# yuyuyu-bot/various_image_processings

Hardware: AMD Instinct MI355X
Metric: Mpixels/sec bilateral r=7 on 4K RGB; % HBM roofline; 1/2/4/8-GPU scaling (higher is better)
Workload: dtype f32; 1 GPU; bilateral r=7 3840x2160 RGB8; ksize=15, frame=3840x2160, rows_per_rank=2160, data=uniform, parallelism=row-tiled x1

## Files before the change

### include/vip.h

```cpp
#ifndef VIP_H
#define VIP_H

#include <stddef.h>
#include <stdint.h>

#ifdef __cplusplus
extern "C" {
#endif

#define VIP_ABI_VERSION 1

#define VIP_NUMERICS_CUDA 0
#define VIP_NUMERICS_CPP 1

#define VIP_ERR_INVALID_ARGUMENT 10001
#define VIP_ERR_UNSUPPORTED_KSIZE 10002
#define VIP_ERR_ALIASING 10003

typedef struct vip_bilateral_s* vip_bilateral_t;
typedef struct vip_adaptive_s* vip_adaptive_t;
typedef struct vip_texture_s* vip_texture_t;
typedef struct vip_upsample_s* vip_upsample_t;

int vip_abi_version(void);
// ... 55 lines not shown
                                 int row_hi, int free_cus, void* stream);
int vip_bilateral_run_c1(vip_bilateral_t h, const uint8_t* d_src, size_t src_pitch, uint8_t* d_dst, size_t dst_pitch,
                         void* stream);
int vip_joint_bilateral_run_c1(vip_bilateral_t h, const uint8_t* d_src, size_t src_pitch, const uint8_t* d_guide,
                               size_t guide_pitch, int guide_channels, uint8_t* d_dst, size_t dst_pitch,
                               void* stream);
int vip_bilateral_run_rows_c1(vip_bilateral_t h, const uint8_t* d_src, size_t src_pitch, const uint8_t* d_guide,
                              size_t guide_pitch, int guide_channels, uint8_t* d_dst, size_t dst_pitch, int out_rows,
                              int src_row0, int row_lo, int row_hi, void* stream);
int vip_joint_bilateral_run_f32(vip_bilateral_t h, const float* d_src, size_t src_pitch, const uint8_t* d_guide,
                                size_t guide_pitch, int guide_channels, float* d_dst, size_t dst_pitch,
                                void* stream);
int vip_joint_bilateral_run_rows_f32(vip_bilateral_t h, const float* d_src, size_t src_pitch,
                                     const uint8_t* d_guide, size_t guide_pitch, int guide_channels, float* d_dst,
                                     size_t dst_pitch, int out_rows, int src_row0, int row_lo, int row_hi,
                                     void* stream);
int vip_joint_bilateral_run_conf_f32(vip_bilateral_t h, const float* d_src, size_t src_pitch, const float* d_conf,
                                     size_t conf_pitch, const uint8_t* d_guide, size_t guide_pitch,
                                     int guide_channels, float hole_value, float* d_dst, size_t dst_pitch,
                                     float* d_weight , size_t weight_pitch, void* stream);
int vip_joint_bilateral_run_f32c(vip_bilateral_t h, const float* d_src, size_t src_pitch, int channels,
                                 const uint8_t* d_guide, size_t guide_pitch, int guide_channels, float* d_dst,
                                 size_t dst_pitch, void* stream);
int vip_upsample_create(vip_upsample_t* out, int width, int height, int scale, int ksize, float sigma_space,
                        float sigma_color, int numerics);
int vip_upsample_destroy(vip_upsample_t h);
int vip_upsample_low_size(int width, int height, int scale, int* low_width, int* low_height);
int vip_upsample_run_f32(vip_upsample_t h, const float* d_src_lo, size_t src_pitch, const uint8_t* d_guide_lo,
                         size_t guide_lo_pitch, const uint8_t* d_guide, size_t guide_pitch, int guide_channels,
                         float* d_dst, size_t dst_pitch, void* stream);
int vip_bilateral_set_waves(int waves);
int vip_bilateral_set_wide(int mode);
int vip_bilateral_set_frames_in_flight(int n);

int vip_adaptive_create(vip_adaptive_t* out, int width, int height, int ksize, float sigma_space, float sigma_color,
                        int numerics);
int vip_adaptive_destroy(vip_adaptive_t h);
int vip_adaptive_run(vip_adaptive_t h, const uint8_t* d_src, size_t src_pitch, uint8_t* d_dst, size_t dst_pitch,
                     void* stream);
int vip_adaptive_run_rows(vip_adaptive_t h, const uint8_t* d_src, size_t src_pitch, uint8_t* d_dst, size_t dst_pitch,
                          int out_rows, int src_row0, int row_lo, int row_hi, void* stream);
int vip_adaptive_run_rows_batch(vip_adaptive_t h, int n, const uint8_t* const* d_srcs, size_t src_pitch,
                                uint8_t* const* d_dsts, size_t dst_pitch, int out_rows, int src_row0, int row_lo,
                                int row_hi, int free_cus, void* stream);
int vip_adaptive_run_c1(vip_adaptive_t h, const uint8_t* d_src, size_t src_pitch, uint8_t* d_dst, size_t dst_pitch,
                        void* stream);
int vip_adaptive_run_rows_c1(vip_adaptive_t h, const uint8_t* d_src, size_t src_pitch, uint8_t* d_dst,
                             size_t dst_pitch, int out_rows, int src_row0, int row_lo, int row_hi, void* stream);

int vip_gradient_u8(const uint8_t* d_src, float* d_dst, int width, int height, int src_ch, int numerics,
                    void* stream);
int vip_gradient_f32(const float* d_src, float* d_dst, int width, int height, int src_ch, int numerics,
                     void* stream);

int vip_texture_create(vip_texture_t* out, int width, int height, int ksize, int nitr, int numerics);
int vip_texture_destroy(vip_texture_t h);
size_t vip_texture_scratch_bytes(int width, int height);
int vip_texture_run(vip_texture_t h, const uint8_t* d_src, uint8_t* d_dst, void* stream);
int vip_texture_run_timed(vip_texture_t h, const uint8_t* d_src, uint8_t* d_dst, void* stream, void* const* events);

#define VIP_TEXTURE_TWO_LAUNCH 0
#define VIP_TEXTURE_FUSED 1
int vip_texture_set_mode(vip_texture_t h, int mode);

int vip_texture_run_c1(vip_texture_t h, const uint8_t* d_src, size_t src_pitch, uint8_t* d_dst, size_t dst_pitch,
                       void* stream);
// ... 14 lines not shown
```

### various_image_processings_amd/_lib.py

```python
from __future__ import annotations

import ctypes
import os
import threading

_HERE = os.path.dirname(os.path.abspath(__file__))
LIB_PATH = os.path.join(_HERE, "libvip_hip.so")

VIP_NUMERICS_CUDA = 0
VIP_NUMERICS_CPP = 1
VIP_ERR_INVALID_ARGUMENT = 10001
VIP_ERR_UNSUPPORTED_KSIZE = 10002
VIP_ERR_ALIASING = 10003
VIP_FILTER_BILATERAL, VIP_FILTER_JOINT, VIP_FILTER_ADAPTIVE, VIP_FILTER_TEXTURE = 0, 1, 2, 3
VIP_FILTER_UPSAMPLE = 4
VIP_FILTER_JOINT_CONF = 5
VIP_FILTER_JOINT_F32C = 6
VIP_PATH_AUTO, VIP_PATH_RUNTIME = 0, 1

_c_void_p = ctypes.c_void_p
_c_int = ctypes.c_int
_c_float = ctypes.c_float
_c_size_t = ctypes.c_size_t

# ... 57 lines not shown
        _c_int, [_c_void_p, _c_void_p, _c_size_t, _c_int, _c_void_p, _c_size_t, _c_int, _c_void_p, _c_size_t,
                 _c_void_p]),
    "vip_joint_f32c_max_ksize": (_c_int, [_c_int]),
    "vip_upsample_create": (
        _c_int, [ctypes.POINTER(_c_void_p), _c_int, _c_int, _c_int, _c_int, _c_float, _c_float, _c_int]),
    "vip_upsample_destroy": (_c_int, [_c_void_p]),
    "vip_upsample_low_size": (_c_int, [_c_int, _c_int, _c_int, ctypes.POINTER(_c_int), ctypes.POINTER(_c_int)]),
    "vip_upsample_run_f32": (
        _c_int, [_c_void_p, _c_void_p, _c_size_t, _c_void_p, _c_size_t, _c_void_p, _c_size_t, _c_int,
                 _c_void_p, _c_size_t, _c_void_p]),
    "vip_adaptive_create": (_c_int, [ctypes.POINTER(_c_void_p), _c_int, _c_int, _c_int, _c_float, _c_float, _c_int]),
    "vip_adaptive_destroy": (_c_int, [_c_void_p]),
    "vip_adaptive_run": (_c_int, [_c_void_p, _c_void_p, _c_size_t, _c_void_p, _c_size_t, _c_void_p]),
    "vip_adaptive_run_rows": (
        _c_int, [_c_void_p, _c_void_p, _c_size_t, _c_void_p, _c_size_t, _c_int, _c_int, _c_int, _c_int, _c_void_p]),
    "vip_adaptive_run_rows_batch": (
        _c_int, [_c_void_p, _c_int, ctypes.POINTER(_c_void_p), _c_size_t, ctypes.POINTER(_c_void_p), _c_size_t,
                 _c_int, _c_int, _c_int, _c_int, _c_int, _c_void_p]),
    "vip_adaptive_run_c1": (_c_int, [_c_void_p, _c_void_p, _c_size_t, _c_void_p, _c_size_t, _c_void_p]),
    "vip_adaptive_run_rows_c1": (
        _c_int, [_c_void_p, _c_void_p, _c_size_t, _c_void_p, _c_size_t, _c_int, _c_int, _c_int, _c_int, _c_void_p]),
    "vip_gradient_u8": (_c_int, [_c_void_p, _c_void_p, _c_int, _c_int, _c_int, _c_int, _c_void_p]),
    "vip_gradient_f32": (_c_int, [_c_void_p, _c_void_p, _c_int, _c_int, _c_int, _c_int, _c_void_p]),
    "vip_texture_create": (_c_int, [ctypes.POINTER(_c_void_p), _c_int, _c_int, _c_int, _c_int, _c_int]),
    "vip_texture_destroy": (_c_int, [_c_void_p]),
    "vip_texture_run": (_c_int, [_c_void_p, _c_void_p, _c_void_p, _c_void_p]),
    "vip_texture_run_timed": (_c_int, [_c_void_p, _c_void_p, _c_void_p, _c_void_p, ctypes.POINTER(_c_void_p)]),
    "vip_texture_run_c1": (_c_int, [_c_void_p, _c_void_p, _c_size_t, _c_void_p, _c_size_t, _c_void_p]),
    "vip_texture_halo_rows": (_c_int, [_c_int]),
    "vip_texture_set_mode": (_c_int, [_c_void_p, _c_int]),
    "vip_bilateral_set_waves": (_c_int, [_c_int]),
    "vip_bilateral_set_wide": (_c_int, [_c_int]),
    "vip_bilateral_set_frames_in_flight": (_c_int, [_c_int]),
    "vip_texture_iterate_rows": (_c_int, [_c_void_p, _c_void_p, _c_void_p, _c_size_t, _c_int, _c_int, _c_int, _c_int,
                                          _c_void_p]),
    "vip_texture_blur_rtv": (_c_int, [_c_void_p, _c_void_p, _c_void_p, _c_void_p, _c_void_p, _c_void_p]),
    "vip_texture_guide": (_c_int, [_c_void_p, _c_void_p, _c_void_p, _c_void_p, _c_void_p]),
}

_lock = threading.Lock()
_lib = None


class VipError(RuntimeError):

    def __init__(self, func: str, code: int):
        self.code = code
        msg = lib().vip_error_string(code).decode()
        super().__init__(f"{func} failed with status {code}: {msg}")


def lib() -> ctypes.CDLL:
    global _lib
    with _lock:
        if _lib is None:
            if not os.path.exists(LIB_PATH):
                raise ImportError(
                    f"{LIB_PATH} is not built; run __graft_entry__.build() "
                    "(make -C various_image_processings_amd/csrc)")
            handle = ctypes.CDLL(LIB_PATH)
            for name, (res, args) in SIGNATURES.items():
                fn = getattr(handle, name)
                fn.restype = res
                fn.argtypes = args
            _lib = handle
    return _lib
# ... 10 lines not shown
```

### various_image_processings_amd/csrc/vip_bilateral.hip

```cpp
#include "vip_launch.hpp"
#include "vip_stencil.hpp"

namespace vip {

#ifdef VIP_STAMPS
__device__ unsigned long long vip_stamps[256 * 16 * 8 * 3];
__device__ __forceinline__ void vip_stamp(int blk, int wave, int t, int k) {
    if ((threadIdx.x & 63) == 0 && t < 8 && blk < 256)
        vip_stamps[((blk * 16 + wave) * 8 + t) * 3 + k] = __builtin_amdgcn_s_memtime();
}
#define VIP_STAMP(t, k) vip_stamp(blockIdx.x, wave, t, k)
__device__ unsigned long long vip_rt[256 * 4];
__device__ __forceinline__ void vip_rt_stamp(int k) {
    if (threadIdx.x == 0 && blockIdx.x < 256) {
        vip_rt[blockIdx.x * 4 + 2 * k] = __builtin_amdgcn_s_memtime();
        vip_rt[blockIdx.x * 4 + 2 * k + 1] = __builtin_amdgcn_s_memrealtime();
    }
}
#define VIP_RT_STAMP(k) vip_rt_stamp(k)
#else
#define VIP_STAMP(t, k)
#define VIP_RT_STAMP(k)
#endif

constexpr int kBilUnrollMaxR = 15;
constexpr bool kBilRcp = true;
template <int R>
struct FoldRank {
    int t[(R + 1) * (R + 1)];
    constexpr FoldRank() : t() {
        for (int y = 0; y <= R; ++y)
            for (int x = 0; x <= R; ++x) t[y * (R + 1) + x] = disc_r2_rank(R, x * x + y * y);
    }
};
constexpr int kPairShareDist = 3;
template <int R, int WAVES, bool JOINT, bool FMA, int COPIES, int P, int NE, bool FOLD, int TPR, bool SAT, bool MULTI>
__device__ __forceinline__ void bilateral_body(const StencilArgs& a) {
    using G = Geom<R, P, TPR>;
    constexpr int NT = WAVES * 64;
    constexpr int TH = WAVES * G::RPW;
    constexpr bool ROW_UNROLL = R <= kBilUnrollMaxR;
    constexpr int ROWS = TH + 2 * R;
    constexpr int PLANE = ROWS * G::S;
    extern __shared__ __attribute__((aligned(16))) uint32_t lds[];
    uint32_t* const lut = lds;
    constexpr int NTAB = FOLD ? disc_r2_count(R) : 1;
    static_assert(SAT == FOLD, "the saturating address serves the folded tables only");
    static_assert(!FOLD || (NE == 32 && COPIES == sat_fold_copies<R>()), "folded tables: saturating address");
    using SL = SatLut<R, 4 * (JOINT ? 2 : 1) * PLANE, disc_r2_count(R), kSatFoldDz, COPIES>;
    uint32_t* const gplane = SAT ? lds + SL::PL / 4 : lds + NTAB * NE * COPIES;
    uint32_t* const splane = JOINT ? gplane + PLANE : gplane;

    const int tid = threadIdx.x;
    const int lane = tid & 63;
    const int wave = __builtin_amdgcn_readfirstlane(tid >> 6);
    const int tx = lane % TPR;
    const int ty = wave * G::RPW + lane / TPR;
    const uint32_t lane4 = (uint32_t)(lane & (COPIES - 1)) << 2;
    const uint32_t sbias = (uint32_t)SL::B0 + lane4;
    const char* const lut_bytes = reinterpret_cast<const char*>(lut);
    const float w0 = __uint_as_float(__builtin_amdgcn_readfirstlane(
        __float_as_uint(FOLD ? a.fold[disc_r2_rank(R, 0) * kFoldEntries] : a.color[0] * a.ws[0])));

    VIP_RT_STAMP(0);
    int tile = blockIdx.x;
    const int items = launch_items<MULTI>(a);
    TilePrefetch<R, ROWS, NT, P, TPR> pg, ps;
    std::conditional_t<SAT, SatStage<NT, SL>, LutStage<NT, NTAB * NE, COPIES>> ls;
    ls.load(FOLD ? a.fold : a.color);
    {
        const FrameTile ft = frame_tile<MULTI>(a, item_tile<MULTI>(a, tile));
        const int tx0 = (ft.t % a.tiles_x) * G::TW, ty0 = (ft.t / a.tiles_x) * TH;
        pg.issue(JOINT ? a.guide : frame_src<MULTI>(a.guide, ft.f), a.guide_pitch, a, tx0, ty0);
        if constexpr (JOINT) ps.issue(a.src, a.src_pitch, a, tx0, ty0);
    }
    ls.store(SAT ? lds + SL::T / 4 : lut);
    pg.commit(gplane);
    if constexpr (JOINT) ps.commit(splane);
    __syncthreads();

    for ([[maybe_unused]] int it = 0;; ++it) {
        VIP_STAMP(it, 0);
        const FrameTile ft = frame_tile<MULTI>(a, item_tile<MULTI>(a, tile));
        const int tx0 = (ft.t % a.tiles_x) * G::TW, ty0 = (ft.t / a.tiles_x) * TH;
        const int next = tile + (int)gridDim.x;
        if (next < items) {
            const FrameTile fn = frame_tile<MULTI>(a, item_tile<MULTI>(a, next));
            const int nx0 = (fn.t % a.tiles_x) * G::TW, ny0 = (fn.t / a.tiles_x) * TH;
            pg.issue(JOINT ? a.guide : frame_src<MULTI>(a.guide, fn.f), a.guide_pitch, a, nx0, ny0);
            if constexpr (JOINT) ps.issue(a.src, a.src_pitch, a, nx0, ny0);
        }
        if (ty0 + wave * G::RPW < a.out_rows && item_wave<MULTI, WAVES>(a, tile, wave)) {
            uint32_t ctr[P];
            {
                const uint4* c = reinterpret_cast<const uint4*>(gplane + (ty + R) * G::S + tx * P + G::L);
#pragma unroll
                for (int q = 0; q < P / 4; ++q) {
                    const uint4 v = c[q];
                    ctr[4 * q + 0] = v.x; ctr[4 * q + 1] = v.y; ctr[4 * q + 2] = v.z; ctr[4 * q + 3] = v.w;
                }
            }
            f2 a01[P], a2k[P];
#pragma unroll
            for (int i = 0; i < P; ++i) a01[i] = a2k[i] = f2{0.f, 0.f};

            for_each_row<R, ROW_UNROLL>([&](const int ky, auto hwc) {
                    constexpr int HW = decltype(hwc)::value;
                    const int aky = ky < 0 ? -ky : ky;
                    set_progress_priority((ky + R) * 4 / (2 * R + 1));
                    const int row_off = (ty + R + ky) * G::S + tx * P;
                    const float* const ws = a.ws + aky * kWsStride;
                    constexpr int C0 = (G::L - HW) / 4, C1 = (G::L + P - 1 + HW) / 4;
                    constexpr int NC = C1 - C0 + 1;
                    float wsv[HW + 1];
#pragma unroll
                    for (int k = 0; k <= HW; ++k) wsv[k] = ws[k];
                    auto widx = [&](uint32_t g, f2, f2, int i, int kx) {
                        uint32_t d = __builtin_amdgcn_sad_u8(g, ctr[i], 0u);
                        if constexpr (FOLD) {
                            constexpr FoldRank<R> rank;
                            return sat_addr(d, SL::S, sbias) + (uint32_t)(SL::T - SL::B0) +
                                   4u * COPIES * rank.t[aky * (R + 1) + (kx < 0 ? -kx : kx)];
                        }
                        return (d << (COPIES == 32 ? 7 : 6)) | lane4;
                    };
// ... 24 lines not shown
        tile = next;
    }
}

template <int R, int WAVES, bool JOINT, bool FMA, int COPIES, int P, int NE = 768, bool FOLD = false, int TPR = 16,
          bool SAT = false>
__global__ __launch_bounds__(WAVES * 64) void bilateral_kernel(const StencilArgs a) {
    bilateral_body<R, WAVES, JOINT, FMA, COPIES, P, NE, FOLD, TPR, SAT, false>(a);
}
template <int R, int WAVES, bool JOINT, bool FMA, int COPIES, int P, int NE = 768, bool FOLD = false, int TPR = 16,
          bool SAT = false>
__global__ __launch_bounds__(WAVES * 64) void bilateral_frames_kernel(const StencilArgs a) {
    bilateral_body<R, WAVES, JOINT, FMA, COPIES, P, NE, FOLD, TPR, SAT, true>(a);
}

constexpr bool kJbfLut16 = true;
constexpr int kJbfP8MaxR = 7;
constexpr int kBilP = 8;
template <int R, int PLANES>
constexpr int outputs_per_thread() { return PLANES == 2 ? (R <= kJbfP8MaxR ? 8 : 4) : kBilP; }
template <int R, int PLANES>
constexpr int lut_copies() {
    constexpr int P = outputs_per_thread<R, PLANES>();
    if (!kJbfLut16 || PLANES == 1) return 32;
    return pick_waves<R, PLANES, 16, 768 * 16, P>() > pick_waves<R, PLANES, 16, 768 * 32, P>() ? 16 : 32;
}

constexpr int kBilSmallMaxR = 8;
constexpr float kWideWork = 0.55f;
struct Tiling {
    int waves;
    bool wide;
};
inline Tiling small_frame_tiling(int width, int out_rows, int inflight = 1, int nframes = 1) {
    const int forced = bilateral_forced_waves();
    const int fwide = bilateral_forced_wide();
    const int share = device_cus() / (inflight > 1 ? inflight : 1);
    const int cus = share > 0 ? share : 1;
    const int cand[3] = {16, 8, 4};
    const float cost[3] = {1.0f, 1.25f, 1.8f};
    Tiling best{16, false};
    float best_t = 0.f;
    bool first = true;
    for (int wide = 0; wide < 2; ++wide) {
        if ((fwide == 1 && wide) || (fwide == 2 && !wide) || (fwide == 0 && forced && wide)) continue;
        const int tw = wide ? 256 : 128, rpw = wide ? 1 : 4;
        const long long tiles_x = (width + tw - 1) / tw;
        for (int i = 0; i < 3; ++i) {
            if (forced && cand[i] != forced) continue;
            const int th = cand[i] * rpw;
            const long long tiles = tiles_x * ((out_rows + th - 1) / th) * (nframes > 1 ? nframes : 1);
            const float t = (float)((tiles + cus - 1) / cus) * cand[i] * cost[i] * (wide ? kWideWork : 1.f);
            if (first || t < best_t) best = Tiling{cand[i], wide != 0}, best_t = t, first = false;
        }
    }
    return best;
}

template <int R, bool JOINT, bool FMA, bool FOLD, int WAVES, bool WIDE = false>
static int launch_bilateral_w(const StencilArgs& a, hipStream_t stream);

template <int R, int WAVES, int PLANES, int P>
constexpr int sat_lds_bytes() {
    return SatLut<R, 4 * PLANES * (WAVES * Geom<R, P>::RPW + 2 * R) * Geom<R, P>::S, disc_r2_count(R), kSatFoldDz,
                  sat_fold_copies<R>()>::BYTES;
}
template <int R, int PLANES, int P>
constexpr int pick_waves_sat() {
    if (sat_lds_bytes<R, 16, PLANES, P>() <= kLdsBudget) return 16;
    if (sat_lds_bytes<R, 12, PLANES, P>() <= kLdsBudget) return 12;
    if (sat_lds_bytes<R, 8, PLANES, P>() <= kLdsBudget) return 8;
    return sat_lds_bytes<R, 4, PLANES, P>() <= kLdsBudget ? 4 : 0;
}

template <int R, bool JOINT, bool FMA, bool FOLD>
static int launch_bilateral_lut(const StencilArgs& a, hipStream_t stream) {
    constexpr int PLANES = JOINT ? 2 : 1;
    constexpr int P = outputs_per_thread<R, PLANES>();
    constexpr int WAVES = FOLD ? pick_waves_sat<R, PLANES, P>()
                               : pick_waves<R, PLANES, 16, 768 * lut_copies<R, PLANES>(), P>();
    static_assert(WAVES > 0, "tile does not fit LDS");
    if constexpr (!JOINT && WAVES == 16 && R <= kBilSmallMaxR) {
        const Tiling t = small_frame_tiling(a.width, a.out_rows, a.inflight, a.nframes);
        if (t.wide) {
            if (t.waves == 16) return launch_bilateral_w<R, JOINT, FMA, FOLD, 16, true>(a, stream);
            if (t.waves == 8) return launch_bilateral_w<R, JOINT, FMA, FOLD, 8, true>(a, stream);
            return launch_bilateral_w<R, JOINT, FMA, FOLD, 4, true>(a, stream);
        }
        if (t.waves == 8) return launch_bilateral_w<R, JOINT, FMA, FOLD, 8>(a, stream);
        if (t.waves == 4) return launch_bilateral_w<R, JOINT, FMA, FOLD, 4>(a, stream);
    }
    return launch_bilateral_w<R, JOINT, FMA, FOLD, WAVES>(a, stream);
}

template <int R, bool JOINT, bool FMA, bool FOLD, int WAVES, bool WIDE>
static int launch_bilateral_w(const StencilArgs& a, hipStream_t stream) {
    static_assert(!FOLD || JOINT, "folded tables: the joint filter");
    static_assert(!WIDE || !JOINT, "wide tiles: the plain filter");
    constexpr int PLANES = JOINT ? 2 : 1;
    constexpr int P = WIDE ? 4 : outputs_per_thread<R, PLANES>();
    constexpr int TPR = WIDE ? 64 : 16;
    using G = Geom<R, P, TPR>;
    constexpr int NE = FOLD ? kFoldEntries : 768;
    constexpr int COPIES = FOLD ? sat_fold_copies<R>() : lut_copies<R, PLANES>();
    constexpr int TH = WAVES * G::RPW;
    constexpr int LDS = FOLD ? sat_lds_bytes<R, WAVES, PLANES, P>() : lds_bytes<R, WAVES, PLANES, NE * COPIES, P, TPR>();
    static_assert(LDS <= kLdsBudget, "tile does not fit LDS");
    constexpr bool SAT = FOLD;
    constexpr auto kern = bilateral_kernel<R, WAVES, JOINT, FMA, COPIES, P, NE, FOLD, TPR, SAT>;
    if constexpr (!JOINT && R <= kBatchMaxRadius) {
        constexpr auto frames_kern = bilateral_frames_kernel<R, WAVES, JOINT, FMA, COPIES, P, NE, FOLD, TPR, SAT>;
        return launch_persistent<kern, frames_kern, LDS, WAVES, G::TW, TH, SAT>(a, a.inflight <= 1, stream);
    } else {
        if (!JOINT && a.nframes > 1) return VIP_ERR_INVALID_ARGUMENT;
        return launch_persistent<kern, nullptr, LDS, WAVES, G::TW, TH, SAT>(a, false, stream);
    }
}

template <int R, bool JOINT, bool FMA>
static int launch_bilateral_r(const StencilArgs& a, hipStream_t stream) {
    if constexpr (JOINT && R <= kSatMaxR)
        if (a.fold && a.lut_nonzero <= SatLut<R, 0, disc_r2_count(R), kSatFoldDz, sat_fold_copies<R>()>::DZ)
            return launch_bilateral_lut<R, JOINT, FMA, true>(a, stream);
    return launch_bilateral_lut<R, JOINT, FMA, false>(a, stream);
}

template <bool JOINT, bool FMA>
static int launch_bilateral_dispatch(int radius, const StencilArgs& a, hipStream_t stream) {
    switch (radius) {
#define VIP_CASE(RR) \
    case RR: return launch_bilateral_r<RR, JOINT, FMA>(a, stream);
#ifdef VIP_ONLY_R7
        VIP_CASE(4) VIP_CASE(7) VIP_CASE(15)
#else
        VIP_CASE(1) VIP_CASE(2) VIP_CASE(3) VIP_CASE(4) VIP_CASE(5) VIP_CASE(6) VIP_CASE(7) VIP_CASE(8)
        VIP_CASE(9) VIP_CASE(10) VIP_CASE(11) VIP_CASE(12) VIP_CASE(13) VIP_CASE(14) VIP_CASE(15)
#endif
#undef VIP_CASE
        default: return VIP_ERR_UNSUPPORTED_KSIZE;
    }
}

#if defined(VIP_BIL_JOINT) && defined(VIP_BIL_FMA)
int launch_bilateral_joint_fma(int radius, const StencilArgs& a, hipStream_t s) {
    return launch_bilateral_dispatch<true, true>(radius, a, s);
}
#elif defined(VIP_BIL_JOINT)
int launch_bilateral_joint_mul(int radius, const StencilArgs& a, hipStream_t s) {
    return launch_bilateral_dispatch<true, false>(radius, a, s);
}
#elif defined(VIP_BIL_FMA)
int launch_bilateral_plain_fma(int radius, const StencilArgs& a, hipStream_t s) {
    return launch_bilateral_dispatch<false, true>(radius, a, s);
}
#ifdef VIP_STAMPS
}
extern "C" int vip_debug_read_stamps(void* host, size_t bytes) {
    return (int)hipMemcpyFromSymbol(host, HIP_SYMBOL(vip::vip_stamps), bytes, 0, hipMemcpyDeviceToHost);
}
extern "C" int vip_debug_read_rt(void* host, size_t bytes) {
    return (int)hipMemcpyFromSymbol(host, HIP_SYMBOL(vip::vip_rt), bytes, 0, hipMemcpyDeviceToHost);
}
namespace vip {
#endif
#else
int launch_bilateral_plain_mul(int radius, const StencilArgs& a, hipStream_t s) {
    return launch_bilateral_dispatch<false, false>(radius, a, s);
}
#endif

}
```

### various_image_processings_amd/csrc/vip_capi.hip

```cpp
#include <atomic>
#include <cmath>
#include <cstdlib>
#include <cstdio>
#include <cstring>
#include <cxxabi.h>
#include <dlfcn.h>
#include <new>
#include <string>
#include <vector>

#include "vip_launch.hpp"

namespace vip {
static int launch_stencil(int filter, int radius, bool fma, const StencilArgs& a, hipStream_t s) {
    if (filter == VIP_FILTER_JOINT)
        return fma ? launch_bilateral_joint_fma(radius, a, s) : launch_bilateral_joint_mul(radius, a, s);
    if (filter == VIP_FILTER_ADAPTIVE) return fma ? launch_adaptive_fma(radius, a, s) : launch_adaptive_mul(radius, a, s);
    return fma ? launch_bilateral_plain_fma(radius, a, s) : launch_bilateral_plain_mul(radius, a, s);
}

static float space_weight(int r2, float sigma_space, int numerics) {
    const float two_s2 = 2 * sigma_space * sigma_space;
    const float cf = -1.f / two_s2;
    const double cd = -1. / (double)two_s2;
// ... 393 lines not shown
        case VIP_FILTER_UPSAMPLE: return kMaxKsizeUpsample;
        case VIP_FILTER_JOINT_CONF: return kMaxKsizeJointConf;
        case VIP_FILTER_JOINT_F32C: return kMaxKsizeJointF32c[2];
        default: return VIP_ERR_INVALID_ARGUMENT;
    }
}

int vip_joint_f32c_max_ksize(int channels) {
    return channels >= 1 && channels <= 4 ? kMaxKsizeJointF32c[channels] : VIP_ERR_INVALID_ARGUMENT;
}

int vip_set_stencil_path(int path) {
    if (path != VIP_PATH_AUTO && path != VIP_PATH_RUNTIME) return VIP_ERR_INVALID_ARGUMENT;
    g_stencil_path.store(path, std::memory_order_relaxed);
    return 0;
}

int vip_bilateral_set_waves(int waves) {
    if (!valid_waves(waves)) return VIP_ERR_INVALID_ARGUMENT;
    g_bil_waves.store(waves, std::memory_order_relaxed);
    return 0;
}

int vip_bilateral_set_wide(int mode) {
    if (mode < 0 || mode > 2) return VIP_ERR_INVALID_ARGUMENT;
    g_bil_wide.store(mode, std::memory_order_relaxed);
    return 0;
}

int vip_bilateral_set_frames_in_flight(int n) {
    if (n < 0 || n > 4) return VIP_ERR_INVALID_ARGUMENT;
    g_bil_inflight.store(n, std::memory_order_relaxed);
    return 0;
}

const char* vip_error_string(int code) {
    switch (code) {
        case 0: return "success";
        case VIP_ERR_INVALID_ARGUMENT: return "invalid argument";
        case VIP_ERR_UNSUPPORTED_KSIZE:
            return "unsupported ksize (odd, 1..65 bilateral, 1..47 joint bilateral, 1..63 adaptive, 1..9 upsampling, 1..31 confidence-weighted "
                   "joint, 1..31 / 1..15 joint on 2 / 3-4 f32 channels; texture 1..24)";
        case VIP_ERR_ALIASING: return "source and destination alias";
        default: return hipGetErrorString((hipError_t)code);
    }
}

int vip_malloc(void** d_ptr, size_t bytes) {
    if (!d_ptr) return VIP_ERR_INVALID_ARGUMENT;
    return (int)hipMalloc(d_ptr, bytes);
}
int vip_free(void* d_ptr) { return (int)hipFree(d_ptr); }
int vip_upload(void* d_dst, const void* h_src, size_t bytes) {
    return (int)hipMemcpy(d_dst, h_src, bytes, hipMemcpyHostToDevice);
}
int vip_download(void* h_dst, const void* d_src, size_t bytes) {
    return (int)hipMemcpy(h_dst, d_src, bytes, hipMemcpyDeviceToHost);
}
int vip_device_synchronize(void) { return (int)hipDeviceSynchronize(); }
int vip_device_count(int* count) {
    if (!count) return VIP_ERR_INVALID_ARGUMENT;
    return (int)hipGetDeviceCount(count);
}
int vip_set_device(int device) { return (int)hipSetDevice(device); }
int vip_get_device(int* device) {
    if (!device) return VIP_ERR_INVALID_ARGUMENT;
// ... 592 lines not shown
```

### various_image_processings_amd/csrc/vip_launch.hpp

```cpp
#pragma once

#include <atomic>
#include <type_traits>
#include <utility>

#include <hip/hip_ext.h>

#include "vip_common.hpp"

namespace vip {

constexpr int kMaxRadius = 15;
constexpr int kWsStride = kMaxRadius + 1;
constexpr int kP = 8;
constexpr int kTW = 16 * kP;
constexpr int kLdsBudget = 160 * 1024;
constexpr int kSatMaxR = 6;
constexpr int kFoldEntries = 32;

constexpr int kMaxBatchFrames = 6;
constexpr int kBatchMaxRadius = 8;

struct StencilArgs {
    const uint8_t* src;
// ... 11 lines not shown
    const float* color;
    int lut_nonzero;
    const float* fold;
    int inflight;
    int nframes;
    int tiles_frame;
    int free_cus;
    int tail_full, tail_shift;
    const uint8_t* fsrc[kMaxBatchFrames];
    uint8_t* fdst[kMaxBatchFrames];
    float ws[kWsStride * kWsStride];
};

constexpr int kRtMaxRadius = 32;

struct RtArgs {
    const uint8_t* src;
    const uint8_t* guide;
    uint8_t* dst;
    long long src_pitch, guide_pitch, dst_pitch;
    int width, out_rows, src_row0, row_lo, row_hi;
    int aligned, dst_aligned;
    const float* color;
    const float* wsrow;
    const int* hw;
    int R, wst, ra;
    int L, S, tiles_x;
};

int launch_bilateral_joint_fma(int radius, const StencilArgs& a, hipStream_t s);
int launch_bilateral_joint_mul(int radius, const StencilArgs& a, hipStream_t s);
int launch_bilateral_plain_fma(int radius, const StencilArgs& a, hipStream_t s);
int launch_bilateral_plain_mul(int radius, const StencilArgs& a, hipStream_t s);
int launch_adaptive_fma(int radius, const StencilArgs& a, hipStream_t s);
int launch_adaptive_mul(int radius, const StencilArgs& a, hipStream_t s);
int launch_stencil_rt(const RtArgs& a, bool joint, bool adaptive, bool fma, hipStream_t stream);
int launch_gray(int radius, int guide_channels, bool fma, const StencilArgs& a, hipStream_t s);
int launch_gray_rt(const RtArgs& a, int guide_channels, bool fma, hipStream_t s);
int launch_gray_adaptive(int radius, bool fma, const StencilArgs& a, hipStream_t s);
int launch_gray_adaptive_rt(const RtArgs& a, bool fma, hipStream_t s);
constexpr int kF32GuideWords = 1;
constexpr int kF32SrcVec = 2;
int launch_joint_f32(int radius, int guide_channels, bool fma, const StencilArgs& a, hipStream_t s);
int launch_joint_f32_rt(const RtArgs& a, int guide_channels, bool fma, hipStream_t s);
constexpr int kUpMaxRadius = 4;
constexpr int kUpGuideWords = 4;
struct UpsampleArgs {
    const uint8_t* src;
    const uint8_t* guide_lo;
    const uint8_t* guide;
    uint8_t* dst;
    long long src_pitch, guide_lo_pitch, guide_pitch, dst_pitch;
    int width, out_rows;
    int low_width, low_height;
    int tiles_x, tiles_total;
    int aligned, dst_aligned;
    const float* color;
    const float* wsp;
};
int launch_upsample_f32(int radius, int scale, int guide_channels, bool fma, const UpsampleArgs& a, hipStream_t s);
struct ConfArgs : StencilArgs {
    const uint8_t* conf;
    uint8_t* weight;
    long long conf_pitch, weight_pitch;
    float hole_value;
    int conf_vec;
// ... 136 lines not shown
```

### various_image_processings_amd/csrc/vip_stencil.hpp

```cpp
#pragma once

#include <type_traits>
#include <utility>

#include "vip_exact.hpp"
#include "vip_launch.hpp"

namespace vip {

constexpr int kSatFoldDz = kFoldEntries - 1;
static_assert(kSatFoldDz < kFoldEntries, "folded tables hold d < kFoldEntries");

template <int R, int PB, int NTAB_ = disc_r2_count(R), int DZMAX = kSatFoldDz, int COPIES_ = 32>
struct SatLut {
    static constexpr int NTAB = NTAB_;
    static constexpr int COPIES = COPIES_;
    static constexpr int S = NTAB * 4 * COPIES;
    static constexpr int LAST = 4 * (COPIES - 1);
    static constexpr int DZ = (65535 - LAST) / S < DZMAX ? (65535 - LAST) / S : DZMAX;
    static constexpr int B0 = 65535 - DZ * S - LAST;
    static constexpr int T = round_up(B0, 16);
    static constexpr int PL = PB <= B0 ? 0 : round_up(T + (DZ + 1) * S, 16);
    static constexpr int BYTES = PB <= B0 ? T + (DZ + 1) * S : PL + PB;
    static_assert(COPIES == 16 || COPIES == 32, "copies");
    static_assert(DZ >= 0 && T - B0 + (NTAB - 1) * 4 * COPIES <= 65535, "ds_read immediate range");
};
template <int R>
constexpr int sat_fold_copies() { return R <= 6 ? 32 : 16; }
static_assert(SatLut<6, 0>::DZ >= 25 && SatLut<8, 0, disc_r2_count(8), kSatFoldDz, 16>::DZ >= 25 &&
                  SatLut<7, 0, disc_r2_count(7), kSatFoldDz, 32>::DZ < 25,
              "folded tables reach the texture JBF's zero point (d = 25) with sat_fold_copies");

constexpr int lut_words(bool adaptive) { return adaptive ? 1536 * 16 : 768 * 32; }

__device__ __forceinline__ int xcd_tile(int slot, int total) {
    const int grid = (int)gridDim.x, b = (int)blockIdx.x;
    const int base = slot - b;
    if ((grid & 7) != 0 || base + grid > total) return slot;
    return base + (b & 7) * (grid >> 3) + (b >> 3);
}

template <int R, int P = kP, int TPR = 16>
struct Geom {
    static_assert((P == 8 && TPR == 16) || (P == 4 && (TPR == 16 || TPR == 64)), "P, TPR");
    static constexpr int TW = TPR * P;
    static constexpr int RPW = 64 / TPR;
    static constexpr int L = round_up(R, 4);
    static constexpr int S = P == 8 ? round_up(TW + 2 * L, 8) + 4
                                    : (TPR == 64 ? round_up(TW + 2 * L, 4) : round_up(TW + 2 * L, 64));
    static constexpr int GROUPS = (TW + 2 * L) / 4;
};

template <int R, int WAVES, int PLANES, int LUTW = lut_words(false), int P = kP, int TPR = 16>
constexpr int lds_bytes() {
    return 4 * LUTW + 4 * PLANES * (WAVES * Geom<R, P, TPR>::RPW + 2 * R) * Geom<R, P, TPR>::S;
}

template <int R, int PLANES, int MAXW = 16, int LUTW = lut_words(false), int P = kP, int TPR = 16>
constexpr int pick_waves() {
    if (MAXW >= 16 && lds_bytes<R, 16, PLANES, LUTW, P, TPR>() <= kLdsBudget) return 16;
    if (MAXW >= 12 && lds_bytes<R, 12, PLANES, LUTW, P, TPR>() <= kLdsBudget) return 12;
    if (MAXW >= 8 && lds_bytes<R, 8, PLANES, LUTW, P, TPR>() <= kLdsBudget) return 8;
    return MAXW >= 4 && lds_bytes<R, 4, PLANES, LUTW, P, TPR>() <= kLdsBudget ? 4 : 0;
}

template <int R, int KY>
struct HwDispatch {
    template <class F>
    __device__ __forceinline__ static void run(int hw, F&& f) {
        constexpr int H = circle_hw(R, KY);
        if constexpr (KY == 0 || circle_hw(R, KY - 1) != H) {
            if (hw == H) {
                f(std::integral_constant<int, H>{});
                return;
            }
        }
        if constexpr (KY < R) HwDispatch<R, KY + 1>::run(hw, static_cast<F&&>(f));
    }
};

template <int R, bool UNROLL, class F>
__device__ __forceinline__ void for_each_row(F&& f) {
    if constexpr (UNROLL) {
        [&]<int... I>(std::integer_sequence<int, I...>) {
// ... 5 lines not shown
            const int aky = ky < 0 ? -ky : ky;
            HwDispatch<R, 0>::run(circle_hw(R, aky), [&](auto hwc) { f(ky, hwc); });
        }
    }
}

__device__ __forceinline__ uint4 unpack_rgb4(uint32_t a, uint32_t b, uint32_t c) {
    uint4 r;
    r.x = a & 0xffffffu;
    r.y = __builtin_amdgcn_alignbyte(b, a, 3) & 0xffffffu;
    r.z = __builtin_amdgcn_alignbyte(c, b, 2) & 0xffffffu;
    r.w = c >> 8;
    return r;
}

__device__ __forceinline__ uint32_t load_rgb(const uint8_t* row, int x) {
    const uint8_t* p = row + 3 * x;
    return (uint32_t)p[0] | ((uint32_t)p[1] << 8) | ((uint32_t)p[2] << 16);
}

template <int N, int K>
__device__ __forceinline__ void win_sum(const uint32_t (&x)[N + K - 1], uint32_t (&o)[N]) {
    uint32_t s = x[0];
#pragma unroll
    for (int k = 1; k < K; ++k) s += x[k];
    o[0] = s;
#pragma unroll
    for (int j = 1; j < N; ++j) {
        s = s + x[j + K - 1] - x[j - 1];
        o[j] = s;
    }
}

template <int R, int ROWS, int NT, int P = kP, int TPR = 16>
struct TilePrefetch {
    using G = Geom<R, P, TPR>;
    static constexpr int NG = ROWS * G::GROUPS;
    static constexpr int K = (NG + NT - 1) / NT;
    uint32_t raw[K][3];

    __device__ __forceinline__ void issue(const uint8_t* img, long long pitch, const StencilArgs& a, int tx0,
                                          int ty0) {
#pragma unroll
        for (int k = 0; k < K; ++k) {
            const int g = (int)threadIdx.x + k * NT;
            if (NG % NT != 0 && k == K - 1 && g >= NG) continue;
            const int r = g / G::GROUPS;
            const int gc = g - r * G::GROUPS;
            const int sy = clampi(ty0 + a.src_row0 - R + r, a.row_lo, a.row_hi - 1);
            const uint8_t* row = img + (long long)sy * pitch;
            const int x = tx0 - G::L + 4 * gc;
            if (a.aligned && x >= 0 && x + 3 < a.width) {
                const uint32_t* w = reinterpret_cast<const uint32_t*>(row + 3 * x);
                raw[k][0] = w[0];
                raw[k][1] = w[1];
                raw[k][2] = w[2];
            } else {
                const uint32_t q0 = load_rgb(row, clampi(x + 0, 0, a.width - 1));
                const uint32_t q1 = load_rgb(row, clampi(x + 1, 0, a.width - 1));
                const uint32_t q2 = load_rgb(row, clampi(x + 2, 0, a.width - 1));
                const uint32_t q3 = load_rgb(row, clampi(x + 3, 0, a.width - 1));
                raw[k][0] = q0 | (q1 << 24);
                raw[k][1] = (q1 >> 8) | (q2 << 16);
                raw[k][2] = (q2 >> 16) | (q3 << 8);
            }
        }
    }

    __device__ __forceinline__ void commit(uint32_t* plane) const {
// ... 150 lines not shown
    for (int j = J0; j <= J1; ++j) {
        if (j + LA <= J1 && ((j + LA) & 3) == 0 && chunk(j + LA) > PRE) row.load(chunk(j + LA));
        if (j + D <= J1) issue(j + D);
        const int b = (j - J0) % NB;
#pragma unroll
        for (int i = 0; i < P; ++i) {
            const int kx = j - L - i;
            if (kx < -HW || kx > HW) continue;
            float w;
            if (own(j, kx) && kx == 0) {
                w = w0;
            } else if (own(j, kx) && kx > 0) {
                w = pw[i][j - L];
            } else {
                w = FOLD ? wc[b][i] : wc[b][i] * wsv[kx < 0 ? -kx : kx];
                if (own(j, kx)) pw[j - L][i] = w;
            }
            if constexpr (FMA) {
                a01[i].x = __builtin_fmaf(n01[b].x, w, a01[i].x);
                a01[i].y = __builtin_fmaf(n01[b].y, w, a01[i].y);
                a2k[i].x = __builtin_fmaf(n21[b].x, w, a2k[i].x);
                a2k[i].y = a2k[i].y + w;
            } else {
                a01[i].x = a01[i].x + n01[b].x * w;
                a01[i].y = a01[i].y + n01[b].y * w;
                a2k[i].x = a2k[i].x + n21[b].x * w;
                a2k[i].y = a2k[i].y + w;
            }
        }
        __builtin_amdgcn_sched_barrier(0);
    }
}

template <int P, bool RCP = false>
__device__ __forceinline__ void finish_outputs(const f2 (&a01)[P], const f2 (&a2k)[P], uint32_t (&o)[P]) {
#pragma unroll
    for (int i = 0; i < P; ++i) {
        const float sk = a2k[i].y;
        if constexpr (RCP) {
            const float y = recip_exact(sk);
            o[i] = f2u8(div_by_sumk(a01[i].x, sk, y) + 0.5f) | (f2u8(div_by_sumk(a01[i].y, sk, y) + 0.5f) << 8) |
                   (f2u8(div_by_sumk(a2k[i].x, sk, y) + 0.5f) << 16);
        } else {
            o[i] = f2u8(a01[i].x / sk + 0.5f) | (f2u8(a01[i].y / sk + 0.5f) << 8) | (f2u8(a2k[i].x / sk + 0.5f) << 16);
        }
    }
}

struct FrameTile {
    int f, t;
};
template <bool MULTI>
__device__ __forceinline__ FrameTile frame_tile(const StencilArgs& a, int mt) {
    int f = 0;
    if constexpr (!MULTI) return {f, mt};
    while (mt >= a.tiles_frame && a.tiles_frame > 0 && f < kMaxBatchFrames - 1) {
        mt -= a.tiles_frame;
        ++f;
    }
    return {f, mt};
}
template <class T>
__device__ __forceinline__ T kernarg_at(size_t byte_offset) {
    typedef const __attribute__((address_space(4))) char kchar;
    typedef const __attribute__((address_space(4))) T kT;
    kchar* base = (kchar*)__builtin_amdgcn_kernarg_segment_ptr();
// ... 86 lines not shown
```

Baseline: 49200 Mpixels/s.

## Compute bilateral outputs as 4x2 patches per thread, sharing symmetric weights

For plain bilateral with radius 5 or 7, each thread now computes a 4-wide by 2-tall patch of outputs instead of an 8-wide row, using a new patch geometry. Range weights between pixels inside the patch, both within a row and across the two rows, are computed once and reused by symmetry, which removes redundant LUT lookups and multiplies. Each loaded neighbour row feeds two output rows. A tile planning API is added to report the chosen tiling. The cost is more registers per thread and a different tile shape, which may change occupancy and how the frame's tiles are balanced across CUs.

```diff
diff --git a/include/vip.h b/include/vip.h
--- a/include/vip.h
+++ b/include/vip.h
@@ -111,6 +111,7 @@
 int vip_bilateral_set_waves(int waves);
 int vip_bilateral_set_wide(int mode);
 int vip_bilateral_set_frames_in_flight(int n);
+int vip_bilateral_plan_tiles(int ksize, int width, int rows, int frames_in_flight, int nframes, int out[6]);
 
 int vip_adaptive_create(vip_adaptive_t* out, int width, int height, int ksize, float sigma_space, float sigma_color,
                         int numerics);
diff --git a/various_image_processings_amd/_lib.py b/various_image_processings_amd/_lib.py
--- a/various_image_processings_amd/_lib.py
+++ b/various_image_processings_amd/_lib.py
@@ -113,6 +113,7 @@
     "vip_bilateral_set_waves": (_c_int, [_c_int]),
     "vip_bilateral_set_wide": (_c_int, [_c_int]),
     "vip_bilateral_set_frames_in_flight": (_c_int, [_c_int]),
+    "vip_bilateral_plan_tiles": (_c_int, [_c_int, _c_int, _c_int, _c_int, _c_int, ctypes.POINTER(_c_int)]),
     "vip_texture_iterate_rows": (_c_int, [_c_void_p, _c_void_p, _c_void_p, _c_size_t, _c_int, _c_int, _c_int, _c_int,
                                           _c_void_p]),
     "vip_texture_blur_rtv": (_c_int, [_c_void_p, _c_void_p, _c_void_p, _c_void_p, _c_void_p, _c_void_p]),
diff --git a/various_image_processings_amd/csrc/vip_bilateral.hip b/various_image_processings_amd/csrc/vip_bilateral.hip
--- a/various_image_processings_amd/csrc/vip_bilateral.hip
+++ b/various_image_processings_amd/csrc/vip_bilateral.hip
@@ -34,9 +34,14 @@
     }
 };
 constexpr int kPairShareDist = 3;
+constexpr bool bil_patch_radius(int r) { return r == 5 || r == 7; }
+template <int R, bool JOINT, int P, int TPR, bool FOLD>
+constexpr bool bil_patch() { return !JOINT && !FOLD && P == 8 && TPR == 16 && bil_patch_radius(R); }
+constexpr int kPatchCrossDist = 3;
 template <int R, int WAVES, bool JOINT, bool FMA, int COPIES, int P, int NE, bool FOLD, int TPR, bool SAT, bool MULTI>
 __device__ __forceinline__ void bilateral_body(const StencilArgs& a) {
-    using G = Geom<R, P, TPR>;
+    constexpr bool PATCH = bil_patch<R, JOINT, P, TPR, FOLD>();
+    using G = std::conditional_t<PATCH, PatchGeom<R>, Geom<R, P, TPR>>;
     constexpr int NT = WAVES * 64;
     constexpr int TH = WAVES * G::RPW;
     constexpr bool ROW_UNROLL = R <= kBilUnrollMaxR;
@@ -55,7 +60,7 @@
     const int lane = tid & 63;
     const int wave = __builtin_amdgcn_readfirstlane(tid >> 6);
     const int tx = lane % TPR;
-    const int ty = wave * G::RPW + lane / TPR;
+    const int ty = wave * G::RPW + (PATCH ? 2 : 1) * (lane / TPR);
     const uint32_t lane4 = (uint32_t)(lane & (COPIES - 1)) << 2;
     const uint32_t sbias = (uint32_t)SL::B0 + lane4;
     const char* const lut_bytes = reinterpret_cast<const char*>(lut);
@@ -65,7 +70,7 @@
     VIP_RT_STAMP(0);
     int tile = blockIdx.x;
     const int items = launch_items<MULTI>(a);
-    TilePrefetch<R, ROWS, NT, P, TPR> pg, ps;
+    TilePrefetch<R, ROWS, NT, P, TPR, G> pg, ps;
     std::conditional_t<SAT, SatStage<NT, SL>, LutStage<NT, NTAB * NE, COPIES>> ls;
     ls.load(FOLD ? a.fold : a.color);
     {
@@ -90,7 +95,32 @@
             pg.issue(JOINT ? a.guide : frame_src<MULTI>(a.guide, fn.f), a.guide_pitch, a, nx0, ny0);
             if constexpr (JOINT) ps.issue(a.src, a.src_pitch, a, nx0, ny0);
         }
-        if (ty0 + wave * G::RPW < a.out_rows && item_wave<MULTI, WAVES>(a, tile, wave)) {
+        if constexpr (PATCH) {
+            if (ty0 + wave * G::RPW < a.out_rows && item_wave<MULTI, WAVES>(a, tile, wave)) {
+                uint32_t ctr[P];
+#pragma unroll
+                for (int r = 0; r < 2; ++r) {
+                    const uint4 v = *reinterpret_cast<const uint4*>(gplane + (ty + r + R) * G::S + tx * 4 + G::L);
+                    ctr[4 * r + 0] = v.x; ctr[4 * r + 1] = v.y; ctr[4 * r + 2] = v.z; ctr[4 * r + 3] = v.w;
+                }
+                f2 a01[P], a2k[P];
+#pragma unroll
+                for (int i = 0; i < P; ++i) a01[i] = a2k[i] = f2{0.f, 0.f};
+                float xw[4][4];
+                [&]<int... I>(std::integer_sequence<int, I...>) {
+                    ((set_progress_priority(I * 4 / (2 * R + 2)),
+                      patch_row_taps<R, I - R, G::L, FMA, COPIES, kPatchCrossDist>(
+                          gplane, (ty + I) * G::S + tx * 4, a.ws, lut_bytes, lane4, ctr, a01, a2k, w0, xw),
+                      fence_accumulators(a01, a2k), __builtin_amdgcn_sched_barrier(0)), ...);
+                }(std::make_integer_sequence<int, 2 * R + 2>{});
+                uint32_t o[P];
+                finish_outputs<P, kBilRcp>(a01, a2k, o);
+                uint8_t* const dst = frame_dst<MULTI>(a, tile);
+                const uint32_t o0[4] = {o[0], o[1], o[2], o[3]}, o1[4] = {o[4], o[5], o[6], o[7]};
+                store_px_to(a, dst, ty0 + ty, tx0 + tx * 4, o0);
+                store_px_to(a, dst, ty0 + ty + 1, tx0 + tx * 4, o1);
+            }
+        } else if (ty0 + wave * G::RPW < a.out_rows && item_wave<MULTI, WAVES>(a, tile, wave)) {
             uint32_t ctr[P];
             {
                 const uint4* c = reinterpret_cast<const uint4*>(gplane + (ty + R) * G::S + tx * P + G::L);
@@ -181,7 +211,8 @@
     int waves;
     bool wide;
 };
-inline Tiling small_frame_tiling(int width, int out_rows, int inflight = 1, int nframes = 1) {
+inline Tiling small_frame_tiling(int width, int out_rows, int inflight = 1, int nframes = 1, int ntw = 128,
+                                 int nrpw = 4) {
     const int forced = bilateral_forced_waves();
     const int fwide = bilateral_forced_wide();
     const int share = device_cus() / (inflight > 1 ? inflight : 1);
@@ -193,7 +224,7 @@
     bool first = true;
     for (int wide = 0; wide < 2; ++wide) {
         if ((fwide == 1 && wide) || (fwide == 2 && !wide) || (fwide == 0 && forced && wide)) continue;
-        const int tw = wide ? 256 : 128, rpw = wide ? 1 : 4;
+        const int tw = wide ? 256 : ntw, rpw = wide ? 1 : nrpw;
         const long long tiles_x = (width + tw - 1) / tw;
         for (int i = 0; i < 3; ++i) {
             if (forced && cand[i] != forced) continue;
@@ -204,6 +235,14 @@
         }
     }
     return best;
+}
+
+template <int R>
+using PlainNarrowGeom = std::conditional_t<bil_patch<R, false, kBilP, 16, false>(), PatchGeom<R>, Geom<R, kBilP, 16>>;
+template <int R>
+inline Tiling plain_tiling(int width, int out_rows, int inflight, int nframes) {
+    if constexpr (R > kBilSmallMaxR) return Tiling{16, false};
+    else return small_frame_tiling(width, out_rows, inflight, nframes, PlainNarrowGeom<R>::TW, PlainNarrowGeom<R>::RPW);
 }
 
 template <int R, bool JOINT, bool FMA, bool FOLD, int WAVES, bool WIDE = false>
@@ -230,7 +269,7 @@
                                : pick_waves<R, PLANES, 16, 768 * lut_copies<R, PLANES>(), P>();
     static_assert(WAVES > 0, "tile does not fit LDS");
     if constexpr (!JOINT && WAVES == 16 && R <= kBilSmallMaxR) {
-        const Tiling t = small_frame_tiling(a.width, a.out_rows, a.inflight, a.nframes);
+        const Tiling t = plain_tiling<R>(a.width, a.out_rows, a.inflight, a.nframes);
         if (t.wide) {
             if (t.waves == 16) return launch_bilateral_w<R, JOINT, FMA, FOLD, 16, true>(a, stream);
             if (t.waves == 8) return launch_bilateral_w<R, JOINT, FMA, FOLD, 8, true>(a, stream);
@@ -249,11 +288,15 @@
     constexpr int PLANES = JOINT ? 2 : 1;
     constexpr int P = WIDE ? 4 : outputs_per_thread<R, PLANES>();
     constexpr int TPR = WIDE ? 64 : 16;
-    using G = Geom<R, P, TPR>;
+    constexpr bool PATCH = bil_patch<R, JOINT, P, TPR, FOLD>();
+    using G = std::conditional_t<PATCH, PatchGeom<R>, Geom<R, P, TPR>>;
     constexpr int NE = FOLD ? kFoldEntries : 768;
     constexpr int COPIES = FOLD ? sat_fold_copies<R>() : lut_copies<R, PLANES>();
+    static_assert(!PATCH || COPIES == 32, "patch kernels: the 768 x 32 LUT (patch_lds_bytes)");
     constexpr int TH = WAVES * G::RPW;
-    constexpr int LDS = FOLD ? sat_lds_bytes<R, WAVES, PLANES, P>() : lds_bytes<R, WAVES, PLANES, NE * COPIES, P, TPR>();
+    constexpr int LDS = PATCH  ? patch_lds_bytes<R>(WAVES)
+                        : FOLD ? sat_lds_bytes<R, WAVES, PLANES, P>()
+                               : lds_bytes<R, WAVES, PLANES, NE * COPIES, P, TPR>();
     static_assert(LDS <= kLdsBudget, "tile does not fit LDS");
     constexpr bool SAT = FOLD;
     constexpr auto kern = bilateral_kernel<R, WAVES, JOINT, FMA, COPIES, P, NE, FOLD, TPR, SAT>;
@@ -302,6 +345,19 @@
 int launch_bilateral_plain_fma(int radius, const StencilArgs& a, hipStream_t s) {
     return launch_bilateral_dispatch<false, true>(radius, a, s);
 }
+int plan_bilateral_plain(int radius, int width, int out_rows, int inflight, int nframes, int* out) {
+    return dispatch_radius(radius, [&](auto rc) {
+        constexpr int R = decltype(rc)::value;
+        using GN = PlainNarrowGeom<R>;
+        using GW = Geom<R, 4, 64>;
+        const Tiling t = plain_tiling<R>(width, out_rows, inflight, nframes);
+        const int tw = t.wide ? GW::TW : GN::TW, th = t.waves * (t.wide ? GW::RPW : GN::RPW);
+        out[0] = t.waves, out[1] = t.wide, out[2] = tw, out[3] = th;
+        out[4] = ((width + tw - 1) / tw) * ((out_rows + th - 1) / th) * nframes;
+        out[5] = 4 * lut_words(false) + 4 * (th + 2 * R) * (t.wide ? GW::S : GN::S);
+        return 0;
+    });
+}
 #ifdef VIP_STAMPS
 }
 extern "C" int vip_debug_read_stamps(void* host, size_t bytes) {
diff --git a/various_image_processings_amd/csrc/vip_capi.hip b/various_image_processings_amd/csrc/vip_capi.hip
--- a/various_image_processings_amd/csrc/vip_capi.hip
+++ b/various_image_processings_amd/csrc/vip_capi.hip
@@ -449,6 +449,13 @@
     if (n < 0 || n > 4) return VIP_ERR_INVALID_ARGUMENT;
     g_bil_inflight.store(n, std::memory_order_relaxed);
     return 0;
+}
+
+int vip_bilateral_plan_tiles(int ksize, int width, int rows, int frames_in_flight, int nframes, int out[6]) {
+    if (!out || width <= 0 || rows <= 0 || frames_in_flight < 1 || nframes < 1 || nframes > vip::kMaxBatchFrames)
+        return VIP_ERR_INVALID_ARGUMENT;
+    if (ksize < 3 || ksize % 2 == 0) return VIP_ERR_UNSUPPORTED_KSIZE;
+    return vip::plan_bilateral_plain(ksize / 2, width, rows, frames_in_flight, nframes, out);
 }
 
 const char* vip_error_string(int code) {
diff --git a/various_image_processings_amd/csrc/vip_launch.hpp b/various_image_processings_amd/csrc/vip_launch.hpp
--- a/various_image_processings_amd/csrc/vip_launch.hpp
+++ b/various_image_processings_amd/csrc/vip_launch.hpp
@@ -67,6 +67,7 @@
 int launch_bilateral_joint_mul(int radius, const StencilArgs& a, hipStream_t s);
 int launch_bilateral_plain_fma(int radius, const StencilArgs& a, hipStream_t s);
 int launch_bilateral_plain_mul(int radius, const StencilArgs& a, hipStream_t s);
+int plan_bilateral_plain(int radius, int width, int out_rows, int inflight, int nframes, int* out);
 int launch_adaptive_fma(int radius, const StencilArgs& a, hipStream_t s);
 int launch_adaptive_mul(int radius, const StencilArgs& a, hipStream_t s);
 int launch_stencil_rt(const RtArgs& a, bool joint, bool adaptive, bool fma, hipStream_t stream);
diff --git a/various_image_processings_amd/csrc/vip_stencil.hpp b/various_image_processings_amd/csrc/vip_stencil.hpp
--- a/various_image_processings_amd/csrc/vip_stencil.hpp
+++ b/various_image_processings_amd/csrc/vip_stencil.hpp
@@ -43,6 +43,7 @@
 template <int R, int P = kP, int TPR = 16>
 struct Geom {
     static_assert((P == 8 && TPR == 16) || (P == 4 && (TPR == 16 || TPR == 64)), "P, TPR");
+    static constexpr int PW = P;
     static constexpr int TW = TPR * P;
     static constexpr int RPW = 64 / TPR;
     static constexpr int L = round_up(R, 4);
@@ -50,6 +51,20 @@
                                     : (TPR == 64 ? round_up(TW + 2 * L, 4) : round_up(TW + 2 * L, 64));
     static constexpr int GROUPS = (TW + 2 * L) / 4;
 };
+
+template <int R>
+struct PatchGeom {
+    static constexpr int PW = 4, PH = 2;
+    static constexpr int TW = 16 * PW;
+    static constexpr int RPW = 4 * PH;
+    static constexpr int L = round_up(R, 4);
+    static constexpr int S = round_up(TW + 2 * L, 32);
+    static constexpr int GROUPS = (TW + 2 * L) / 4;
+};
+template <int R>
+constexpr int patch_lds_bytes(int waves) {
+    return 4 * lut_words(false) + 4 * (waves * PatchGeom<R>::RPW + 2 * R) * PatchGeom<R>::S;
+}
 
 template <int R, int WAVES, int PLANES, int LUTW = lut_words(false), int P = kP, int TPR = 16>
 constexpr int lds_bytes() {
@@ -121,9 +136,9 @@
     }
 }
 
-template <int R, int ROWS, int NT, int P = kP, int TPR = 16>
+template <int R, int ROWS, int NT, int P = kP, int TPR = 16, class G_ = Geom<R, P, TPR>>
 struct TilePrefetch {
-    using G = Geom<R, P, TPR>;
+    using G = G_;
     static constexpr int NG = ROWS * G::GROUPS;
     static constexpr int K = (NG + NT - 1) / NT;
     uint32_t raw[K][3];
@@ -340,6 +355,102 @@
     }
 }
 
+template <int R, int K, int L, bool FMA, int COPIES, int CROSS, int D = kPipeDepth>
+__device__ __forceinline__ void patch_row_taps(const uint32_t* plane, int row_off, const float* ws, const char* lut,
+                                               uint32_t lane4, const uint32_t (&ctr)[8], f2 (&a01)[8],
+                                               f2 (&a2k)[8], const float w0, float (&xw)[4][4]) {
+    constexpr int PW = 4;
+    constexpr int KY0 = K, KY1 = K - 1;
+    constexpr int AK0 = KY0 < 0 ? -KY0 : KY0, AK1 = KY1 < 0 ? -KY1 : KY1;
+    constexpr int HW0 = AK0 <= R ? circle_hw(R, AK0 <= R ? AK0 : 0) : -1;
+    constexpr int HW1 = AK1 <= R ? circle_hw(R, AK1 <= R ? AK1 : 0) : -1;
+    constexpr int HW = HW0 > HW1 ? HW0 : HW1;
+    static_assert(HW >= 0 && L >= HW, "neighbour row of the patch");
+    constexpr int NB = D + 1;
+    constexpr int J0 = L - HW;
+    constexpr int J1 = L + PW - 1 + HW;
+    constexpr int C0 = J0 / 4, NC = J1 / 4 - C0 + 1;
+    constexpr int LA = D + kRowLookahead;
+    auto chunk = [](int j) constexpr { return (j - 4 * C0) >> 2; };
+    constexpr int PRE = chunk(J0 + LA < J1 ? J0 + LA : J1);
+    RowStream<C0, NC, false> row(plane, plane, row_off);
+#pragma unroll
+    for (int q = 0; q <= PRE; ++q) row.load(q);
+    float wsv0[R + 1], wsv1[R + 1];
+#pragma unroll
+    for (int k = 0; k <= HW0; ++k) wsv0[k] = ws[AK0 * kWsStride + k];
+#pragma unroll
+    for (int k = 0; k <= HW1; ++k) wsv1[k] = ws[AK1 * kWsStride + k];
+    enum { NONE, LUT, KEEP_PAIR, KEEP_CROSS, TAKE_PAIR, TAKE_CROSS, CENTRE };
+    auto kind = [](int j, int r, int c) constexpr {
+        const int kx = j - L - c, akx = kx < 0 ? -kx : kx;
+        const int hw = r ? HW1 : HW0, ky = r ? KY1 : KY0;
+        if (akx > hw) return (int)NONE;
+        if (j < L || j >= L + PW) return (int)LUT;
+        if (ky == 0) return kx == 0 ? (int)CENTRE : kx < 0 ? (int)KEEP_PAIR : (int)TAKE_PAIR;
+        if (r == 1 && ky == -1 && akx <= CROSS) return (int)KEEP_CROSS;
+        if (r == 0 && ky == 1 && akx <= CROSS) return (int)TAKE_CROSS;
+        return (int)LUT;
+    };
+    float wc[NB][8];
+    f2 n01[NB], n21[NB];
+    [[maybe_unused]] float pw[PW][PW];
+    auto issue = [&](int j) {
+        const uint32_t g = row.guide(j - 4 * C0);
+        const int b = (j - J0) % NB;
+        n01[b].x = (float)(g & 0xffu);
+        n01[b].y = (float)((g >> 8) & 0xffu);
+        n21[b].x = (float)((g >> 16) & 0xffu);
+        n21[b].y = 1.0f;
+#pragma unroll
+        for (int i = 0; i < 2 * PW; ++i) {
+            const int k = kind(j, i / PW, i % PW);
+            if (k != LUT && k != KEEP_PAIR && k != KEEP_CROSS) continue;
+            const uint32_t d = __builtin_amdgcn_sad_u8(g, ctr[i], 0u);
+            wc[b][i] = *reinterpret_cast<const float*>(lut + ((d << (COPIES == 32 ? 7 : 6)) | lane4));
+        }
+    };
+#pragma unroll
+    for (int j = J0; j < J0 + D && j <= J1; ++j) issue(j);
+#pragma unroll
+    for (int j = J0; j <= J1; ++j) {
+        if (j + LA <= J1 && ((j + LA) & 3) == 0 && chunk(j + LA) > PRE) row.load(chunk(j + LA));
+        if (j + D <= J1) issue(j + D);
+        const int b = (j - J0) % NB;
+#pragma unroll
+        for (int i = 0; i < 2 * PW; ++i) {
+            const int r = i / PW, c = i % PW;
+            const int k = kind(j, r, c);
+            if (k == NONE) continue;
+            const int kx = j - L - c, akx = kx < 0 ? -kx : kx;
+            float w;
+            if (k == CENTRE) {
+                w = w0;
+            } else if (k == TAKE_PAIR) {
+                w = pw[c][j - L];
+            } else if (k == TAKE_CROSS) {
+                w = xw[c][j - L];
+            } else {
+                w = wc[b][i] * (r ? wsv1[akx] : wsv0[akx]);
+                if (k == KEEP_PAIR) pw[j - L][c] = w;
+                if (k == KEEP_CROSS) xw[j - L][c] = w;
+            }
+            if constexpr (FMA) {
+                a01[i].x = __builtin_fmaf(n01[b].x, w, a01[i].x);
+                a01[i].y = __builtin_fmaf(n01[b].y, w, a01[i].y);
+                a2k[i].x = __builtin_fmaf(n21[b].x, w, a2k[i].x);
+                a2k[i].y = a2k[i].y + w;
+            } else {
+                a01[i].x = a01[i].x + n01[b].x * w;
+                a01[i].y = a01[i].y + n01[b].y * w;
+                a2k[i].x = a2k[i].x + n21[b].x * w;
+                a2k[i].y = a2k[i].y + w;
+            }
+        }
+        __builtin_amdgcn_sched_barrier(0);
+    }
+}
+
 template <int P, bool RCP = false>
 __device__ __forceinline__ void finish_outputs(const f2 (&a01)[P], const f2 (&a2k)[P], uint32_t (&o)[P]) {
 #pragma unroll
```

New measurement: 49680 Mpixels/s (median of 4 runs). About the same (+1.0%).
